# Twinklebear/tray_rust

Measured on AMD Instinct MI355X. Metric: Msamples/s (whole node) at 1920x1080; achieved HBM GB/s vs peak, higher is better.
Workload: dtype f32

## Files before the change

### tray_rust_amd/csrc/hip/dev_integrator.h

```cpp
#pragma once
#include "dev_tex.h"

#ifdef TR_LEAN_TILES
#ifndef TR_LEAN_PICK
#define TR_LEAN_MIS_PDF_FIRST
#endif
#endif

namespace tr {

template <int ANIM>
TR_DEV Ray camera_ray(const DevScene& sc, float px, float py, float time) {
    const TrayCamera& c = *sc.camera_p;
    f3 q = xf_point(c.raster_to_cam, mk(px, py, 0.0f));
    f3 px_pos = mk(c.scaling[0], c.scaling[1], c.scaling[2]) * q;
    f3 d = normalized(px_pos);
    const float frame_time = (c.shutter_close - c.shutter_open) * time + c.shutter_open;
    Ray r;
    if (ANIM && c.animated) {
        float x[TR_XF_WORDS];
        if (ANIM == 1 && sc.xf_tab) {
            const float4* __restrict__ rec = reinterpret_cast<const float4*>(sc.xf_tab + ((size_t)xf_time_index(time) * sc.xf_tab_stride + sc.n_moving) * TR_XF_REC);
#pragma unroll
            for (int q = 0; q < TR_XF_WORDS / 4; ++q) { const float4 v = rec[q]; x[4 * q] = v.x; x[4 * q + 1] = v.y; x[4 * q + 2] = v.z; x[4 * q + 3] = v.w; }
        } else
        eval_xform_stack(sc.xf_levels, sc.keyframes, sc.knots, c.xf_first, c.xf_count, frame_time, x);
        r.o = xf_point_affine_w(x, x[25], mk(0.0f, 0.0f, 0.0f));
        r.d = xf_vector(x, d);
    } else {
        r.o = xf_point(c.cam_world, mk(0.0f, 0.0f, 0.0f));
        r.d = xf_vector(c.cam_world, d);
    }
    r.min_t = 0.0f; r.max_t = TR_INF;
    r.time = frame_time; r.col = 0u;
    return r;
}

TR_DEV void pixel_sample(uint32_t kp, uint32_t s, uint32_t spp, uint32_t px, uint32_t py, float& x, float& y, float& t) {
    uint32_t idx = permute(s, spp, draw(kp, PD_PERM_XY));
    x = van_der_corput(idx, draw(kp, PD_SCR_X)) + (float)px;
    y = sobol(idx, draw(kp, PD_SCR_Y)) + (float)py;
    t = van_der_corput(permute(s, spp, draw(kp, PD_PERM_T)), draw(kp, PD_SCR_T));
}

TR_DEV float rr_draw(uint32_t ks, uint32_t bounce) { return (float)(draw(ks, SD_RR + bounce) >> 8) / 16777216.0f; }

template <int ANIM>
TR_DEV f3 inst_emission(const DevScene& sc, const TrayInstance* __restrict__ in, float time) {
    if (ANIM && in->emis_count >= 2u) return color_keys_at(sc.color_keys + in->emis_first, in->emis_count, time);
    return mk(in->emission[0], in->emission[1], in->emission[2]);
}
template <int ANIM>
TR_DEV f3 emitter_radiance(const DevScene& sc, const TrayInstance* __restrict__ in, f3 w, f3 n, float time) {
    return dot(w, n) > 0.0f ? inst_emission<ANIM>(sc, in, time) : mk(0.0f, 0.0f, 0.0f);
}

enum : uint32_t {
    LF_ALIVE = 1u,
    LF_SPECULAR = 2u,
    LF_SHADOW = 4u,
    LF_MIS = 8u,
    LF_LAST = 16u,
    LF_MIS_MISS = 1024u,
    LF_MIS_UNTESTED = 2048u
};
enum : uint32_t { WANT_NONE = 0, WANT_LIGHT = 1, WANT_MIS = 2, WANT_PATH = 3 };

struct Lane {
    uint32_t flags;
    uint32_t bounce;
    uint32_t ks;
    float time;
    uint32_t col;
    f3 d;
#define LN_O(ln) ((ln).bsdf.p)
    f3 throughput, illum;
    f3 first_ng;
    Bsdf bsdf;
    uint32_t light_inst;
    f3 li;
    union { f3 wi_l; f3 mis_f; };
    float pdf_l;
    f3 aux_d;
    f3 direct;
    f3 t_vertex;
    LdsB perm_lds = nullptr;
    uint32_t smp_kind = TRAY_SAMPLER_LOW_DISCREPANCY, smp_offset = 0u;
#ifdef TR_STAGE_CLOCKS
    unsigned long long* qclk = nullptr;
    long long qt = 0;
#endif
};
#ifdef TR_STAGE_CLOCKS
#define TR_QCLK_START(ln) do { if ((ln).qclk) (ln).qt = clock64(); } while (0)
#define TR_QCLK(ln, k) do { if ((ln).qclk) { const long long n_ = clock64(); (ln).qclk[k] += (unsigned long long)(n_ - (ln).qt); (ln).qt = n_; } } while (0)
#else
#define TR_QCLK_START(ln) ((void)0)
#define TR_QCLK(ln, k) ((void)0)
#endif

TR_DEV void lane_start_sample(Lane& ln, const Ray& cam_ray, uint32_t ks) {
    ln.flags = LF_ALIVE;
    ln.bounce = 0u;
    ln.ks = ks;
    LN_O(ln) = cam_ray.o; ln.d = cam_ray.d;
    ln.time = cam_ray.time; ln.col = 0u;
    ln.throughput = mk(1.0f, 1.0f, 1.0f);
    ln.illum = mk(0.0f, 0.0f, 0.0f);
}

TR_DEV uint32_t lane_perm_entry(const DevScene& sc, const Lane& ln, uint32_t s1, uint32_t s2) {
    const uint32_t off1 = ((s1 & (TR_PERM_POOL - 1u)) << 4) + ln.bounce;
    const uint32_t e1 = ln.perm_lds ? (uint32_t)ln.perm_lds[off1] : (uint32_t)sc.perm_pool[off1];
    const uint32_t off2 = ((s2 & (TR_PERM_POOL - 1u)) << 4) + (__brev(e1 >> 4) >> 28);
    return ln.perm_lds ? (uint32_t)ln.perm_lds[off2] : (uint32_t)sc.perm_pool[off2];
}
TR_DEV float lane_uniform(const Lane& ln, uint32_t dim, uint32_t c) {
    return (float)(draw(ln.ks, 64u + 32u * dim + 2u * ln.bounce + c) >> 8) / 16777216.0f;
}
TR_DEV void lane_2d(const DevScene& sc, const Lane& ln, uint32_t dim, float& u0, float& u1) {
    if (ln.smp_kind == TRAY_SAMPLER_UNIFORM) { u0 = lane_uniform(ln, dim, 0u); u1 = lane_uniform(ln, dim, 1u); return; }
    const uint32_t sx = draw(ln.ks, dim), sy = draw(ln.ks, dim + 1u);
    const uint32_t e = lane_perm_entry(sc, ln, sx, sy);
    if (ln.smp_kind == TRAY_SAMPLER_ADAPTIVE) {
        const uint32_t idx = (__brev(e >> 4) >> 28) + ln.smp_offset;
        u0 = van_der_corput(idx, sx); u1 = sobol(idx, sy);
        return;
    }
    u0 = u24_to_unit(((e & 0xf0u) << 24) ^ sx);
    u1 = u24_to_unit((e << 28) ^ sy);
}
TR_DEV float lane_1d(const DevScene& sc, const Lane& ln, uint32_t dim) {
    if (ln.smp_kind == TRAY_SAMPLER_UNIFORM) return lane_uniform(ln, dim, 0u);
    const uint32_t s = draw(ln.ks, dim);
    const uint32_t e = lane_perm_entry(sc, ln, s, s >> 8);
    if (ln.smp_kind == TRAY_SAMPLER_ADAPTIVE) return van_der_corput((__brev(e >> 4) >> 28) + ln.smp_offset, s);
    return u24_to_unit(((e & 0xf0u) << 24) ^ s);
}

TR_DEV Ray stage_a_ray(const Lane& ln) {
    Ray r;
    r.o = LN_O(ln); r.d = ln.d;
    r.min_t = ln.bounce == 0u ? 0.0f : 0.001f;
    r.max_t = TR_INF;
    r.time = ln.time; r.col = ln.col;
    return r;
}
TR_DEV Ray stage_b_ray(const Lane& ln) {
    Ray r;
    r.o = ln.bsdf.p; r.d = ln.aux_d; r.min_t = 0.001f; r.max_t = 0.999f;
    r.time = ln.time; r.col = ln.col;
    return r;
}
TR_DEV Ray stage_c_ray(const Lane& ln) {
    Ray r;
    r.o = ln.bsdf.p; r.d = ln.aux_d; r.min_t = 0.001f; r.max_t = TR_INF;
    r.time = ln.time; r.col = ln.col;
    return r;
}

template <int ANIM>
TR_DEV void vertex_begin(const DevScene& sc, Lane& ln, const HitRec& rec, Counters& cnt) {
    cnt.vertices++;
    const Ray ray = stage_a_ray(ln);
    Hit hit = finish_hit<ANIM>(sc, ray, rec);
    if (ln.bounce == 0u) ln.first_ng = hit.ng;
    const TrayInstance* __restrict__ inst = sc.instances + hit.inst;
    if (ln.bounce == 0u || (ln.flags & LF_SPECULAR)) {
        if (inst->kind != TRAY_INST_RECEIVER) {
            f3 w = -ln.d;
            ln.illum = ln.illum + ln.throughput * emitter_radiance<ANIM>(sc, inst, w, ln.first_ng, ln.time);
        }
    }
    ln.bsdf = make_bsdf(sc, hit);
    if (sc.integrator == TRAY_INTEGRATOR_NORMALS_DEBUG) {
        ln.illum = (ln.bsdf.n + mk(1.0f, 1.0f, 1.0f)) / 2.0f;
        ln.flags &= ~(LF_ALIVE | LF_SHADOW | LF_MIS | LF_MIS_MISS | LF_MIS_UNTESTED);
        return;
    }
    ln.direct = mk(0.0f, 0.0f, 0.0f);
    ln.t_vertex = ln.throughput;
    ln.flags &= ~(LF_SHADOW | LF_MIS | LF_LAST | LF_MIS_MISS | LF_MIS_UNTESTED);
    float l1 = lane_1d(sc, ln, SD_L1);
    float fl = l1 * (float)sc.n_lights;
    uint32_t li_idx = fl > 0.0f ? (uint32_t)fl : 0u;
    if (li_idx > sc.n_lights - 1u) li_idx = sc.n_lights - 1u;
    ln.light_inst = sc.lights[li_idx];
    const TrayInstance* __restrict__ light = sc.instances + ln.light_inst;
    f3 p_w;
    float x[TR_XF_WORDS];
    if (ANIM) instance_xf_at<ANIM>(sc, light, ln.time, ln.col, x);
    if (light->kind == TRAY_INST_POINT_EMITTER) {
        f3 pos = ANIM ? xf_point_affine_w(x, x[25], mk(0.0f, 0.0f, 0.0f)) : xf_point(light->mat, mk(0.0f, 0.0f, 0.0f));
        ln.wi_l = normalized(pos - ln.bsdf.p);
        ln.li = inst_emission<ANIM>(sc, light, ln.time) / length_sqr(pos - ln.bsdf.p);
        ln.pdf_l = 1.0f;
        p_w = pos;
    } else {
        float l2x, l2y;
        lane_2d(sc, ln, SD_L2, l2x, l2y);
        f3 p_l = ANIM ? xf_point_affine_w(x + 12, x[24], ln.bsdf.p) : xf_point(light->inv, ln.bsdf.p);
        f3 p_sampled, normal;
        geom_sample(light, p_l, l2x, l2y, p_sampled, normal);
        f3 w_il = normalized(p_sampled - p_l);
        ln.pdf_l = geom_pdf(light, p_l, w_il);
        ln.li = emitter_radiance<ANIM>(sc, light, -w_il, normal, ln.time);
        p_w = ANIM ? xf_point_affine_w(x, x[25], p_sampled) : xf_point(light->mat, p_sampled);
        ln.wi_l = ANIM ? xf_vector(x, w_il) : xf_vector(light->mat, w_il);
    }
    if (ln.pdf_l > 0.0f && !is_black(ln.li)) {
        ln.aux_d = p_w - ln.bsdf.p;
        ln.flags |= LF_SHADOW;
    }
}

// ... 192 lines not shown
```

### tray_rust_amd/csrc/hip/kernel_tiles.hip

```cpp
#ifndef TR_TILES_GROUP
#error "compile with -DTR_TILES_GROUP=<0 | 1> (csrc/Makefile)"
#endif
#define TR_DEVICE_TU
#define TR_LEAN_TILES
#include "kernels.hip"
#include "kernel_select.h"
#include "kernel_tiles.h"

namespace tr_tiles {

#if TR_TILES_GROUP == 0
void path_tiles(int feat, bool light_filter, dim3 grid, dim3 block, size_t lds, hipStream_t stream, const tr::DevScene& dev, const uint2* tiles,
                uint32_t tile_count, uint32_t chunk, uint32_t chunk_stride, uint32_t spp, uint32_t kf, uint32_t levels, float* rgbw, uint32_t* counter,
                DevStats* stats) {
    if (feat != FEAT_NONE) { path_tiles_lobes(feat, light_filter, grid, block, lds, stream, dev, tiles, tile_count, chunk, chunk_stride, spp, kf, levels, rgbw, counter, stats); return; }
    select_path_tiles_filter<0, FEAT_NONE>(light_filter, [&](auto kernel) {
        hipLaunchKernelGGL(kernel, grid, block, lds, stream, dev, tiles, tile_count, chunk, chunk_stride, spp, kf, levels, rgbw, counter, stats);
    });
}
const void* path_tiles_kernel(int feat, bool light_filter) {
    if (feat != FEAT_NONE) return path_tiles_kernel_lobes(feat, light_filter);
    const void* k = nullptr;
    select_path_tiles_filter<0, FEAT_NONE>(light_filter, [&](auto kernel) { k = reinterpret_cast<const void*>(kernel); });
    return k;
}
#else
template <class F>
static void select_lobes(int feat, bool light_filter, F&& f) {
    if (feat == FEAT_MERL) select_path_tiles_filter<0, FEAT_MERL>(light_filter, f);
    else if (feat == FEAT_SPEC) select_path_tiles_filter<0, FEAT_SPEC>(light_filter, f);
    else if (feat == (FEAT_MERL | FEAT_SPEC)) select_path_tiles_filter<0, FEAT_MERL | FEAT_SPEC>(light_filter, f);
    else if (feat == (FEAT_ALL | FEAT_TEX)) select_path_tiles_filter<0, FEAT_ALL | FEAT_TEX>(light_filter, f);
    else select_path_tiles_filter<0, FEAT_ALL>(light_filter, f);
}
void path_tiles_lobes(int feat, bool light_filter, dim3 grid, dim3 block, size_t lds, hipStream_t stream, const tr::DevScene& dev, const uint2* tiles,
                      uint32_t tile_count, uint32_t chunk, uint32_t chunk_stride, uint32_t spp, uint32_t kf, uint32_t levels, float* rgbw,
                      uint32_t* counter, DevStats* stats) {
    select_lobes(feat, light_filter, [&](auto kernel) {
        hipLaunchKernelGGL(kernel, grid, block, lds, stream, dev, tiles, tile_count, chunk, chunk_stride, spp, kf, levels, rgbw, counter, stats);
    });
}
const void* path_tiles_kernel_lobes(int feat, bool light_filter) {
    const void* k = nullptr;
    select_lobes(feat, light_filter, [&](auto kernel) { k = reinterpret_cast<const void*>(kernel); });
    return k;
}
#endif

}
```

### tray_rust_amd/csrc/hip/kernels.hip

```cpp
#ifndef TR_HOST_EMU
#include <hip/hip_runtime.h>
#endif
#include <stdint.h>

#include <cstdio>
#include <cstdlib>
#include <cstring>
#include <mutex>
#include <thread>
#include <dlfcn.h>
#include <string>
#include <type_traits>
#include <utility>
#include <algorithm>
#include <vector>

#include "../../../include/trayhip.h"
#include "../host/validate.hpp"
#include "dev_integrator.h"
#include "dev_whitted.h"

namespace trayh { void set_error(const std::string& msg); }
using trayh::set_error;
using namespace tr;
// ... 139 lines not shown
                                                       int x0, int y0, int py_l, float sx, float sy, f3 c) {
    const float img_x = sx - 0.5f, img_y = sy - 0.5f;
    const float e8 = (img_y - (float)(y0 + py_l)) * 8.0f;
    const float fl8 = floorf(e8);
    if (e8 == fl8 || fl8 < -4.0f || fl8 > 3.0f) { film_splat_global(sc, rgbw, s_table, x0, y0, sx, sy, c); return; }
    const int cy = (int)fl8 + 4;
    const int fpw = sc.fpw;
    const int xr0 = max(x0 - fpw, 0), xr1 = min(x0 + 8 + fpw, (int)sc.width - 1);
    int ix_lo, ix_hi;
    film_admit(sx, xr0, xr1, fpw, ix_lo, ix_hi);
    const int wx0 = x0 - fpw;
    float* __restrict__ row = bins + (py_l * 8 + cy) * ROW_W * 4;
    for (int ix = ix_lo; ix <= ix_hi; ++ix) {
        float fx = fabsf((float)ix - img_x) * sc.inv_w;
        if (fx > sc.filter_w) continue;
        int fx_idx = min((int)(fx * (float)TRAY_FILTER_TABLE_SIZE), TRAY_FILTER_TABLE_SIZE - 1);
        float wx = s_tx[fx_idx];
        float* __restrict__ o = row + (ix - wx0) * 4;
        if (LDS_BINS) {
            atomicAdd(o + 0, wx * c.x); atomicAdd(o + 1, wx * c.y); atomicAdd(o + 2, wx * c.z); atomicAdd(o + 3, wx);
        } else {
            wg_add(o + 0, wx * c.x); wg_add(o + 1, wx * c.y); wg_add(o + 2, wx * c.z); wg_add(o + 3, wx);
        }
    }
}

#include "wavefront.h"

TR_DEV const float* sc_filter_table(const DevScene& sc) { return sc.filter_table; }

template <int ANIM, int FEAT, int INTEG = TRAY_INTEGRATOR_PATH, bool LFILT = false>
__global__ __launch_bounds__(TR_BLOCK, (FEAT == 15 || INTEG != TRAY_INTEGRATOR_PATH) ? TR_MIN_WAVES_SIDE : ANIM ? TR_MIN_WAVES_ANIM : TR_MIN_WAVES) void k_path_tiles(const DevScene scv, const uint2* __restrict__ tiles, uint32_t tile_count,
                                                         uint32_t chunk, uint32_t chunk_stride, uint32_t spp, uint32_t kf, uint32_t levels,
                                                         float* __restrict__ rgbw, uint32_t* __restrict__ counter,
                                                         DevStats* __restrict__ stats
#ifdef TR_SAMPLE_RANGES
                                                         , uint32_t smp_begin = 0u, uint32_t smp_end = 0u
#endif
                                                         ) {
    const float* __restrict__ const s_table = sc_filter_table(scv);
    __shared__ float s_rowbin[ROWBIN_SIZE];
    __shared__ float s_tx[TRAY_FILTER_TABLE_SIZE], s_ty[TRAY_FILTER_TABLE_SIZE];
    __shared__ uint4 s_perm[TR_PERM_BYTES / 16];
    TR_DYN_LDS(uint32_t, s_stack);
    __shared__ uint32_t s_tile, s_next_sample;
    float* const s_win = reinterpret_cast<float*>(s_stack + scv.win_offset);
    const DevScene& sc = scv;
    const DevScene* const scp = &scv;
    const uint32_t tid = threadIdx.x;
    const uint32_t lane = tid & 63u;
    uint32_t* const my_stack = s_stack + tid;
    if (tid < TRAY_FILTER_TABLE_SIZE) { s_tx[tid] = sc.filter_x[tid]; s_ty[tid] = sc.filter_y[tid]; }
    s_perm[tid] = reinterpret_cast<const uint4*>(sc.perm_pool)[tid];
    static_assert(TR_PERM_BYTES / 16 == TR_BLOCK, "one uint4 of the permutation pool per thread");
    const bool film_rows = sc.film_rows != 0u;
    Counters cnt;
    cnt.rays = 0; cnt.vertices = 0;
    uint32_t w_samples = 0u, w_vertices = 0u, w_rays = 0u;
#ifdef TR_STAGE_CLOCKS
    unsigned long long clk[12] = {0, 0, 0, 0, 0, 0, 0, 0, 0, 0, 0, 0};
    long long clk_t = clock64();
#endif
    for (;;) {
        __syncthreads();
        if (tid == 0) { s_tile = atomicAdd(counter, 1u); s_next_sample = 0u; }
        if (film_rows) { for (uint32_t i = tid; i < ROWBIN_SIZE; i += TR_BLOCK) s_rowbin[i] = 0.0f; }
        else for (uint32_t i = tid; i < 4 * WIN_PLANE; i += TR_BLOCK) s_win[i] = 0.0f;
        __syncthreads();
        const uint32_t item = s_tile;
        if (item >= tile_count * levels) break;
        const uint32_t level = item / tile_count, ti = item - level * tile_count, last = levels - 1u;
#ifdef TR_SAMPLE_RANGES
        const uint32_t n_smp = smp_end ? smp_end - smp_begin : spp;
        const uint32_t s_lo = smp_begin + n_smp - (n_smp >> level), s_per_slice = (level < last ? n_smp - (n_smp >> (level + 1u)) : n_smp) - (n_smp - (n_smp >> level));
#else
        const uint32_t s_per_slice = level < last ? spp >> (level + 1u) : spp >> last, s_lo = level < last ? spp - (spp >> level) : spp - (spp >> last);
#endif
        const uint2 tile = tiles[(ti / chunk) * chunk_stride * chunk + (ti % chunk)];
        const int x0 = (int)tile.x * 8, y0 = (int)tile.y * 8;
        const uint32_t n_pairs = 64u * s_per_slice;
        bool pairs_left = true;
        uint32_t row_l = 0u;
        bool pending = false;
        float sx = 0.0f, sy = 0.0f;
#ifdef TR_SAMPLE_DUMP
        size_t dump_idx = 0; uint32_t dump_v = 0u;
#endif
        Lane ln;
        ln.flags = 0u;
        ln.illum = mk(0.0f, 0.0f, 0.0f);
        ln.perm_lds = TR_LDS_B(s_perm);
#ifdef TR_STAGE_CLOCKS
        ln.qclk = clk + 8;
#endif
        for (;;) {
            bool started = false;
            uint32_t kidx = 0u;
            const bool idle = !(ln.flags & LF_ALIVE);
            if (idle && pending) {
#ifdef TR_SAMPLE_DUMP
                if (sc.sample_dump) {
                    sc.sample_dump[2 * dump_idx] = make_float4(ln.illum.x, ln.illum.y, ln.illum.z, (float)dump_v);
                    sc.sample_dump[2 * dump_idx + 1] = make_float4(ln.throughput.x, ln.throughput.y, ln.throughput.z, (float)ln.bounce);
                }
#endif
                if (film_rows) film_splat_rows(sc, s_rowbin, s_tx, rgbw, s_table, x0, y0, (int)row_l, sx, sy, lane_result(ln));
                else film_splat(sc, s_win, s_table, x0, y0, sx, sy, lane_result(ln));
                pending = false;
            }
            const unsigned long long idle_m = __ballot(idle);
            if (pairs_left && idle_m != 0ull) {
                const uint32_t n_idle = (uint32_t)__popcll(idle_m), leader = (uint32_t)__ffsll((long long)idle_m) - 1u;
                uint32_t base = 0u;
                if (lane == leader) base = atomicAdd(&s_next_sample, n_idle);
                base = __shfl(base, (int)leader);
                pairs_left = base + n_idle < n_pairs;
                const uint32_t pair = base + (uint32_t)__popcll(idle_m & ((1ull << lane) - 1ull));
                if (idle && pair < n_pairs) {
#ifdef TR_PAIR_BY_PIXEL
                    const uint32_t pix = pair / s_per_slice, s = s_lo + (pair % s_per_slice);
#else
                    const uint32_t pix = pair & 63u, s = s_lo + (pair >> 6);
#endif
                    const uint32_t px = (uint32_t)x0 + (pix & 7u), py = (uint32_t)y0 + (pix >> 3);
                    const uint32_t kp = key_pixel(kf, py * sc.width + px);
                    float t;
                    pixel_sample(kp, s, spp, px, py, sx, sy, t);
                    lane_start_sample(ln, camera_ray<ANIM>(sc, sx, sy, t), key_sample(kp, s));
                    if (ANIM) { ln.col = xf_cache_lane(); kidx = xf_time_index(t); }
                    row_l = pix >> 3;
                    started = true;
                    pending = true;
#ifdef TR_SAMPLE_DUMP
                    dump_idx = (size_t)(py * sc.width + px) * spp + s; dump_v = 0u;
#endif
                }
            }
            if (ANIM && idle_m != 0ull) xf_cache_fill_wave(sc, started, ln.time, ln.col, kidx);
            w_samples += (uint32_t)__popcll(__ballot(started));
            if (!__any(ln.flags & LF_ALIVE)) break;
            if (INTEG == TRAY_INTEGRATOR_WHITTED) {
                Ray cam;
                cam.o = LN_O(ln); cam.d = ln.d; cam.min_t = 0.0f; cam.max_t = TR_INF; cam.time = ln.time; cam.col = ln.col;
                ln.illum = whitted_run<ANIM>(sc, scp, my_stack, cam, ln.ks, (ln.flags & LF_ALIVE) != 0u, cnt, w_vertices, w_rays);
                ln.flags &= ~LF_ALIVE;
                continue;
            }
#ifdef TR_STAGE_CLOCKS
#define TR_CLK(slot) do { const long long now_ = clock64(); clk[slot] += (unsigned long long)(now_ - clk_t); clk_t = now_; } while (0)
            TR_CLK(6);
#else
#define TR_CLK(slot) ((void)0)
#endif
#pragma nounroll
            for (int stage = 0; stage < 3; ++stage) {
                const bool alive = (ln.flags & LF_ALIVE) != 0u;
                if (LFILT && stage == 2 && alive) mis_ray_filter<ANIM>(sc, ln);
                const bool want_ray = alive && (stage == 0 || (stage == 1 && (ln.flags & LF_SHADOW)) || (stage == 2 && (ln.flags & LF_MIS)));
                TraceResult tr_;
                tr_.hit = false;
                tr_.rec.t = 0.0f; tr_.rec.inst = 0xffffffffu; tr_.rec.prim = 0u; tr_.rec.b1 = 0.0f; tr_.rec.b2 = 0.0f;
                const unsigned long long wr_ = __ballot(want_ray);
                w_rays += (uint32_t)__popcll(wr_);
                if (LFILT && stage == 2) w_rays += (uint32_t)__popcll(__ballot(alive && (ln.flags & LF_MIS_MISS) != 0u));
                if (wr_ != 0ull) {
                    const Ray r = stage == 0 ? stage_a_ray(ln) : (stage == 1 ? stage_b_ray(ln) : stage_c_ray(ln));
                    tr_ = trace<ANIM, LFILT>(scp, my_stack, r, stage == 1, want_ray);
                }
                TR_CLK(stage);
                if (stage == 0) w_vertices += (uint32_t)__popcll(__ballot(alive && tr_.hit));
#ifdef TR_SAMPLE_DUMP
                if (stage == 0 && alive && tr_.hit) ++dump_v;
#endif
                if (stage == 1) {
#ifdef TR_LEAN_MIS_PDF_FIRST
                    vertex_queries<ANIM, FEAT, KM_ALL, !LFILT>(sc, ln, tr_.hit, alive);
#else
                    vertex_queries<ANIM, FEAT>(sc, ln, tr_.hit, alive);
#endif
                } else if (alive) {
                    if (stage == 0) {
                        if (tr_.hit) vertex_begin<ANIM>(sc, ln, tr_.rec, cnt);
                        else ln.flags &= ~LF_ALIVE;
                    } else {
                        if (!vertex_end<ANIM>(sc, ln, tr_.hit, tr_.rec)) ln.flags &= ~LF_ALIVE;
                    }
                }
                TR_CLK(3 + stage);
            }
        }
        __syncthreads();
        if (film_rows) {
            for (uint32_t i = tid; i < 4 * WIN_PLANE; i += TR_BLOCK) s_win[i] = 0.0f;
            __syncthreads();
            film_resolve_rows(sc, s_rowbin, s_ty, s_win, y0, tid);
            __syncthreads();
        }
        const int wx0 = x0 - sc.fpw, wy0 = y0 - sc.fph;
        const int ww = 8 + 2 * sc.fpw + 1, wh = 8 + 2 * sc.fph + 1;
        for (int i = (int)tid; i < ww * wh; i += TR_BLOCK) {
            int wy = i / ww, wx = i - wy * ww;
            int ix = wx0 + wx, iy = wy0 + wy;
            if (ix < 0 || iy < 0 || ix >= (int)sc.width || iy >= (int)sc.height) continue;
            int o = wy * WIN_STRIDE + wx;
            float a = s_win[o + 3 * WIN_PLANE];
            if (a == 0.0f && s_win[o] == 0.0f && s_win[o + WIN_PLANE] == 0.0f && s_win[o + 2 * WIN_PLANE] == 0.0f) continue;
            float* dst = rgbw + ((size_t)iy * sc.width + ix) * 4;
            atomicAdd(dst + 0, s_win[o]);
            atomicAdd(dst + 1, s_win[o + WIN_PLANE]);
            atomicAdd(dst + 2, s_win[o + 2 * WIN_PLANE]);
            atomicAdd(dst + 3, a);
        }
    }
    if (stats) {
        if (lane == 0u) {
            atomicAdd(&stats->samples, (unsigned long long)w_samples);
            atomicAdd(&stats->vertices, (unsigned long long)w_vertices);
            atomicAdd(&stats->rays, (unsigned long long)w_rays);
        }
#ifdef TR_STAGE_CLOCKS
        if ((tid & 63u) == 0u)
            for (int k = 0; k < 11; ++k) atomicAdd(&stats->trav[k], clk[k]);
#endif
    }
}
#undef TR_CLK

#ifndef TR_DEVICE_TU
__global__ __launch_bounds__(TR_BLOCK) void k_xf_table_build(const DevScene scv, float* __restrict__ table, uint32_t stride, uint32_t index0, uint32_t n_index) {
    const DevScene& sc = scv;
    const uint32_t i = blockIdx.x * TR_BLOCK + threadIdx.x, m = blockIdx.y;
    if (i >= n_index) return;
    const uint32_t index = index0 + i;
    const TrayCamera& c = *sc.camera_p;
    const float frame_time = (c.shutter_close - c.shutter_open) * xf_index_time(index) + c.shutter_open;
    uint32_t first, count;
    if (m < sc.n_moving) { const TrayInstance* __restrict__ in = sc.instances + sc.moving_ids[m]; first = in->xf_first; count = in->xf_count; }
    else { first = c.xf_first; count = c.xf_count; }
    float x[TR_XF_WORDS];
    eval_xform_stack(sc.xf_levels, sc.keyframes, sc.knots, first, count, frame_time, x);
    float4* __restrict__ rec = reinterpret_cast<float4*>(table + ((size_t)index * stride + m) * TR_XF_REC);
#pragma unroll
    for (int q = 0; q < TR_XF_WORDS / 4; ++q) rec[q] = make_float4(x[4 * q], x[4 * q + 1], x[4 * q + 2], x[4 * q + 3]);
}
__global__ __launch_bounds__(TR_BLOCK) void k_xf_table_check(const DevScene scv, const float* __restrict__ table, uint32_t stride, uint32_t n, uint32_t* __restrict__ n_bad) {
    const DevScene& sc = scv;
    const uint32_t i = blockIdx.x * TR_BLOCK + threadIdx.x;
    if (i >= n) return;
    uint32_t h = i * 0x9E3779B1u + 0x7feb352du; h ^= h >> 16; h *= 0x846ca68bu; h ^= h >> 15;
    const uint32_t index = h & 0xffffffu, m = (h >> 24) % stride;
    const TrayCamera& c = *sc.camera_p;
    const float frame_time = (c.shutter_close - c.shutter_open) * xf_index_time(index) + c.shutter_open;
    uint32_t first, count;
    if (m < sc.n_moving) { const TrayInstance* __restrict__ in = sc.instances + sc.moving_ids[m]; first = in->xf_first; count = in->xf_count; }
    else { first = c.xf_first; count = c.xf_count; }
    float x[TR_XF_WORDS];
    eval_xform_stack(sc.xf_levels, sc.keyframes, sc.knots, first, count, frame_time, x);
    const uint32_t* __restrict__ rec = reinterpret_cast<const uint32_t*>(table + ((size_t)index * stride + m) * TR_XF_REC);
    bool bad = false;
    for (int q = 0; q < TR_XF_WORDS; ++q) bad = bad || rec[q] != __float_as_uint(x[q]);
    if (bad) atomicAdd(n_bad, 1u);
}
#endif

template <int ANIM>
__global__ __launch_bounds__(TR_BLOCK) void k_debug_intersect(const DevScene scv, uint32_t n, const TrayRay* __restrict__ rays,
                                                              TrayHit* __restrict__ hits) {
    TR_DYN_LDS(uint32_t, s_stack);
    const DevScene& sc = scv;
    const DevScene* const scp = &scv;
    const uint32_t idx = blockIdx.x * blockDim.x + threadIdx.x;
    const bool in_range = idx < n;
    const uint32_t i = in_range ? idx : 0u;
    Ray r;
    r.o = mk(rays[i].o[0], rays[i].o[1], rays[i].o[2]);
    r.d = mk(rays[i].d[0], rays[i].d[1], rays[i].d[2]);
    r.min_t = rays[i].min_t; r.max_t = rays[i].max_t; r.time = rays[i].time; r.col = 0u;
    TrayHit o;
    memset(&o, 0, sizeof o);
    TraceResult tr_ = trace<ANIM>(scp, s_stack + threadIdx.x, r, false, in_range);
    if (!in_range) return;
    const HitRec rec = tr_.rec;
    if (tr_.hit) {
        float uv[2];
        f3 dp_dv;
        Hit h = finish_hit<ANIM>(sc, r, rec, uv, &dp_dv);
        o.t = rec.t; o.inst = rec.inst; o.prim = rec.prim;
        o.p[0] = h.p.x; o.p[1] = h.p.y; o.p[2] = h.p.z;
        o.n[0] = h.n.x; o.n[1] = h.n.y; o.n[2] = h.n.z;
        o.ng[0] = h.ng.x; o.ng[1] = h.ng.y; o.ng[2] = h.ng.z;
        o.u = uv[0]; o.v = uv[1];
        o.dp_du[0] = h.dp_du.x; o.dp_du[1] = h.dp_du.y; o.dp_du[2] = h.dp_du.z;
        o.dp_dv[0] = dp_dv.x; o.dp_dv[1] = dp_dv.y; o.dp_dv[2] = dp_dv.z;
    } else {
        o.t = r.max_t; o.inst = 0xffffffffu;
    }
    hits[i] = o;
}

template <int ANIM>
__global__ __launch_bounds__(TR_BLOCK) void k_debug_sample_radiance(const DevScene scv, uint32_t n, const uint32_t* __restrict__ px,
                                                                    const uint32_t* __restrict__ py, const uint32_t* __restrict__ si,
                                                                    uint32_t spp, uint32_t kf, float* __restrict__ out) {
    TR_DYN_LDS(uint32_t, s_stack);
    const DevScene& sc = scv;
    const DevScene* const scp = &scv;
    const uint32_t idx = blockIdx.x * blockDim.x + threadIdx.x;
    const bool in_range = idx < n;
    const uint32_t i = in_range ? idx : 0u;
    Counters cnt;
    cnt.rays = 0; cnt.vertices = 0;
    const uint32_t kp = key_pixel(kf, py[i] * sc.width + px[i]);
    float sx, sy, t;
    pixel_sample(kp, si[i], spp, px[i], py[i], sx, sy, t);
    Lane ln;
    lane_start_sample(ln, camera_ray<ANIM>(sc, sx, sy, t), key_sample(kp, si[i]));
    if (!in_range) ln.flags = 0u;
    uint32_t* const my_stack = s_stack + threadIdx.x;
    if (sc.integrator == TRAY_INTEGRATOR_WHITTED) {
        Ray cam;
        cam.o = LN_O(ln); cam.d = ln.d; cam.min_t = 0.0f; cam.max_t = TR_INF; cam.time = ln.time; cam.col = ln.col;
        uint32_t wv = 0u, wr = 0u;
        ln.illum = whitted_run<ANIM>(sc, scp, my_stack, cam, ln.ks, in_range, cnt, wv, wr);
        ln.flags = 0u;
    }
    while (__any(ln.flags & LF_ALIVE)) {
#pragma nounroll
        for (int stage = 0; stage < 3; ++stage) {
            const bool alive = (ln.flags & LF_ALIVE) != 0u;
            if (stage == 2 && alive) mis_ray_filter<ANIM>(sc, ln);
            const bool want_ray = alive && (stage == 0 || (stage == 1 && (ln.flags & LF_SHADOW)) || (stage == 2 && (ln.flags & LF_MIS)));
            TraceResult tr_;
            tr_.hit = false;
            tr_.rec.t = 0.0f; tr_.rec.inst = 0xffffffffu; tr_.rec.prim = 0u; tr_.rec.b1 = 0.0f; tr_.rec.b2 = 0.0f;
            if (stage == 2 && alive && (ln.flags & LF_MIS_MISS)) cnt.rays++;
            if (__any(want_ray)) {
                if (want_ray) cnt.rays++;
                const Ray r = stage == 0 ? stage_a_ray(ln) : (stage == 1 ? stage_b_ray(ln) : stage_c_ray(ln));
                tr_ = trace<ANIM>(scp, my_stack, r, stage == 1, want_ray);
            }
// ... 263 lines not shown
```

Measured before the change: 1236.

## Fold sparse MIS rays into the next iteration's primary trace stage

After: 1273 (median of 6 runs). 3.0% higher.

```diff
diff --git a/tray_rust_amd/csrc/hip/dev_integrator.h b/tray_rust_amd/csrc/hip/dev_integrator.h
--- a/tray_rust_amd/csrc/hip/dev_integrator.h
+++ b/tray_rust_amd/csrc/hip/dev_integrator.h
@@ -4,6 +4,11 @@
 #ifdef TR_LEAN_TILES
 #ifndef TR_LEAN_PICK
 #define TR_LEAN_MIS_PDF_FIRST
+#endif
+#endif
+#ifdef TR_LEAN_FOLD_MIS_RAY
+#ifndef TR_LEAN_FOLD_MIN_LANES
+#define TR_LEAN_FOLD_MIN_LANES 8
 #endif
 #endif
 
@@ -61,6 +66,10 @@
     LF_SHADOW = 4u,
     LF_MIS = 8u,
     LF_LAST = 16u,
+#ifdef TR_LEAN_FOLD_MIS_RAY
+    LF_FOLD = 16384u,
+    LF_SIT = 32768u,
+#endif
     LF_MIS_MISS = 1024u,
     LF_MIS_UNTESTED = 2048u
 };
diff --git a/tray_rust_amd/csrc/hip/kernel_fold.h b/tray_rust_amd/csrc/hip/kernel_fold.h
--- /dev/null
+++ b/tray_rust_amd/csrc/hip/kernel_fold.h
@@ -0,0 +1,10 @@
+#pragma once
+
+namespace tr_fold {
+void path_tiles(int feat, dim3 grid, dim3 block, size_t lds, hipStream_t stream, const tr::DevScene& dev, const uint2* tiles, uint32_t tile_count,
+                uint32_t chunk, uint32_t chunk_stride, uint32_t spp, uint32_t kf, uint32_t levels, float* rgbw, uint32_t* counter, DevStats* stats);
+const void* path_tiles_kernel(int feat);
+void path_tiles_lobes(int feat, dim3 grid, dim3 block, size_t lds, hipStream_t stream, const tr::DevScene& dev, const uint2* tiles, uint32_t tile_count,
+                      uint32_t chunk, uint32_t chunk_stride, uint32_t spp, uint32_t kf, uint32_t levels, float* rgbw, uint32_t* counter, DevStats* stats);
+const void* path_tiles_kernel_lobes(int feat);
+}
diff --git a/tray_rust_amd/csrc/hip/kernel_fold.hip b/tray_rust_amd/csrc/hip/kernel_fold.hip
--- /dev/null
+++ b/tray_rust_amd/csrc/hip/kernel_fold.hip
@@ -0,0 +1,47 @@
+#ifndef TR_FOLD_GROUP
+#error "compile with -DTR_FOLD_GROUP=<0 | 1> (csrc/Makefile)"
+#endif
+#define TR_DEVICE_TU
+#define TR_LEAN_TILES
+#if !defined(TR_LEAN_PICK) && !defined(TR_LEAN_FOLD_MIS_RAY)
+#define TR_LEAN_FOLD_MIS_RAY
+#endif
+#include "kernels.hip"
+#include "kernel_fold.h"
+
+namespace tr_fold {
+
+#if TR_FOLD_GROUP == 0
+void path_tiles(int feat, dim3 grid, dim3 block, size_t lds, hipStream_t stream, const tr::DevScene& dev, const uint2* tiles, uint32_t tile_count,
+                uint32_t chunk, uint32_t chunk_stride, uint32_t spp, uint32_t kf, uint32_t levels, float* rgbw, uint32_t* counter, DevStats* stats) {
+    if (feat != FEAT_NONE) { path_tiles_lobes(feat, grid, block, lds, stream, dev, tiles, tile_count, chunk, chunk_stride, spp, kf, levels, rgbw, counter, stats); return; }
+    hipLaunchKernelGGL((k_path_tiles<0, FEAT_NONE, TRAY_INTEGRATOR_PATH, false>), grid, block, lds, stream, dev, tiles, tile_count, chunk, chunk_stride, spp, kf, levels, rgbw,
+                       counter, stats);
+}
+const void* path_tiles_kernel(int feat) {
+    if (feat != FEAT_NONE) return path_tiles_kernel_lobes(feat);
+    return reinterpret_cast<const void*>(k_path_tiles<0, FEAT_NONE, TRAY_INTEGRATOR_PATH, false>);
+}
+#else
+template <class F>
+static void select_lobes(int feat, F&& f) {
+    if (feat == FEAT_MERL) f(k_path_tiles<0, FEAT_MERL, TRAY_INTEGRATOR_PATH, false>);
+    else if (feat == FEAT_SPEC) f(k_path_tiles<0, FEAT_SPEC, TRAY_INTEGRATOR_PATH, false>);
+    else if (feat == (FEAT_MERL | FEAT_SPEC)) f(k_path_tiles<0, FEAT_MERL | FEAT_SPEC, TRAY_INTEGRATOR_PATH, false>);
+    else if (feat == (FEAT_ALL | FEAT_TEX)) f(k_path_tiles<0, FEAT_ALL | FEAT_TEX, TRAY_INTEGRATOR_PATH, false>);
+    else f(k_path_tiles<0, FEAT_ALL, TRAY_INTEGRATOR_PATH, false>);
+}
+void path_tiles_lobes(int feat, dim3 grid, dim3 block, size_t lds, hipStream_t stream, const tr::DevScene& dev, const uint2* tiles, uint32_t tile_count,
+                      uint32_t chunk, uint32_t chunk_stride, uint32_t spp, uint32_t kf, uint32_t levels, float* rgbw, uint32_t* counter, DevStats* stats) {
+    select_lobes(feat, [&](auto kernel) {
+        hipLaunchKernelGGL(kernel, grid, block, lds, stream, dev, tiles, tile_count, chunk, chunk_stride, spp, kf, levels, rgbw, counter, stats);
+    });
+}
+const void* path_tiles_kernel_lobes(int feat) {
+    const void* k = nullptr;
+    select_lobes(feat, [&](auto kernel) { k = reinterpret_cast<const void*>(kernel); });
+    return k;
+}
+#endif
+
+}
diff --git a/tray_rust_amd/csrc/hip/kernel_tiles.hip b/tray_rust_amd/csrc/hip/kernel_tiles.hip
--- a/tray_rust_amd/csrc/hip/kernel_tiles.hip
+++ b/tray_rust_amd/csrc/hip/kernel_tiles.hip
@@ -6,19 +6,27 @@
 #include "kernels.hip"
 #include "kernel_select.h"
 #include "kernel_tiles.h"
+#include "kernel_fold.h"
 
 namespace tr_tiles {
 
 #if TR_TILES_GROUP == 0
+static bool folds() { const char* e = getenv("TRAYHIP_LEAN_FOLD"); return !e || atoi(e) != 0; }
 void path_tiles(int feat, bool light_filter, dim3 grid, dim3 block, size_t lds, hipStream_t stream, const tr::DevScene& dev, const uint2* tiles,
                 uint32_t tile_count, uint32_t chunk, uint32_t chunk_stride, uint32_t spp, uint32_t kf, uint32_t levels, float* rgbw, uint32_t* counter,
                 DevStats* stats) {
+    if (!light_filter && folds()) {
+        if (getenv("TRAYHIP_STATS")) fprintf(stderr, "[trayhip] lean tile kernel: the folding instantiation (libtrayhip_foldmis.so)\n");
+        tr_fold::path_tiles(feat, grid, block, lds, stream, dev, tiles, tile_count, chunk, chunk_stride, spp, kf, levels, rgbw, counter, stats);
+        return;
+    }
     if (feat != FEAT_NONE) { path_tiles_lobes(feat, light_filter, grid, block, lds, stream, dev, tiles, tile_count, chunk, chunk_stride, spp, kf, levels, rgbw, counter, stats); return; }
     select_path_tiles_filter<0, FEAT_NONE>(light_filter, [&](auto kernel) {
         hipLaunchKernelGGL(kernel, grid, block, lds, stream, dev, tiles, tile_count, chunk, chunk_stride, spp, kf, levels, rgbw, counter, stats);
     });
 }
 const void* path_tiles_kernel(int feat, bool light_filter) {
+    if (!light_filter && folds()) return tr_fold::path_tiles_kernel(feat);
     if (feat != FEAT_NONE) return path_tiles_kernel_lobes(feat, light_filter);
     const void* k = nullptr;
     select_path_tiles_filter<0, FEAT_NONE>(light_filter, [&](auto kernel) { k = reinterpret_cast<const void*>(kernel); });
diff --git a/tray_rust_amd/csrc/hip/kernels.hip b/tray_rust_amd/csrc/hip/kernels.hip
--- a/tray_rust_amd/csrc/hip/kernels.hip
+++ b/tray_rust_amd/csrc/hip/kernels.hip
@@ -315,32 +315,76 @@
 #else
 #define TR_CLK(slot) ((void)0)
 #endif
+#ifdef TR_LEAN_FOLD_MIS_RAY
+            constexpr bool FOLD = !LFILT && !ANIM && INTEG == TRAY_INTEGRATOR_PATH;
+            if (FOLD) ln.flags &= ~LF_SIT;
+#endif
 #pragma nounroll
             for (int stage = 0; stage < 3; ++stage) {
+#ifdef TR_LEAN_FOLD_MIS_RAY
+                const bool alive = FOLD ? (ln.flags & (LF_ALIVE | LF_SIT)) == LF_ALIVE : (ln.flags & LF_ALIVE) != 0u;
+#else
                 const bool alive = (ln.flags & LF_ALIVE) != 0u;
+#endif
                 if (LFILT && stage == 2 && alive) mis_ray_filter<ANIM>(sc, ln);
                 const bool want_ray = alive && (stage == 0 || (stage == 1 && (ln.flags & LF_SHADOW)) || (stage == 2 && (ln.flags & LF_MIS)));
                 TraceResult tr_;
                 tr_.hit = false;
                 tr_.rec.t = 0.0f; tr_.rec.inst = 0xffffffffu; tr_.rec.prim = 0u; tr_.rec.b1 = 0.0f; tr_.rec.b2 = 0.0f;
+#ifdef TR_LEAN_FOLD_MIS_RAY
+                unsigned long long wr_ = __ballot(want_ray);
+                if (FOLD && stage == 2 && wr_ != 0ull && (uint32_t)__popcll(wr_) < (uint32_t)(TR_LEAN_FOLD_MIN_LANES)) {
+                    if (want_ray) {
+                        ln.flags |= LF_FOLD;
+#ifdef TR_HOST_EMU
+                        { extern unsigned long long tr_fold_rays; ++tr_fold_rays; }
+#endif
+                    }
+                    wr_ = 0ull;
+                }
+                const bool folded = FOLD && (ln.flags & LF_FOLD) != 0u;
+#else
                 const unsigned long long wr_ = __ballot(want_ray);
+#endif
                 w_rays += (uint32_t)__popcll(wr_);
                 if (LFILT && stage == 2) w_rays += (uint32_t)__popcll(__ballot(alive && (ln.flags & LF_MIS_MISS) != 0u));
                 if (wr_ != 0ull) {
+#ifdef TR_LEAN_FOLD_MIS_RAY
+                    const Ray r = stage == 0 && !folded ? stage_a_ray(ln) : (stage == 1 ? stage_b_ray(ln) : stage_c_ray(ln));
+#else
                     const Ray r = stage == 0 ? stage_a_ray(ln) : (stage == 1 ? stage_b_ray(ln) : stage_c_ray(ln));
+#endif
                     tr_ = trace<ANIM, LFILT>(scp, my_stack, r, stage == 1, want_ray);
                 }
                 TR_CLK(stage);
+#ifdef TR_LEAN_FOLD_MIS_RAY
+                if (stage == 0) w_vertices += (uint32_t)__popcll(__ballot(alive && !folded && tr_.hit));
+#ifdef TR_SAMPLE_DUMP
+                if (stage == 0 && alive && !folded && tr_.hit) ++dump_v;
+#endif
+#else
                 if (stage == 0) w_vertices += (uint32_t)__popcll(__ballot(alive && tr_.hit));
 #ifdef TR_SAMPLE_DUMP
                 if (stage == 0 && alive && tr_.hit) ++dump_v;
 #endif
+#endif
                 if (stage == 1) {
 #ifdef TR_LEAN_MIS_PDF_FIRST
                     vertex_queries<ANIM, FEAT, KM_ALL, !LFILT>(sc, ln, tr_.hit, alive);
 #else
                     vertex_queries<ANIM, FEAT>(sc, ln, tr_.hit, alive);
 #endif
+#ifdef TR_LEAN_FOLD_MIS_RAY
+                } else if (alive) {
+                    if (stage == 0 && !folded) {
+                        if (tr_.hit) vertex_begin<ANIM>(sc, ln, tr_.rec, cnt);
+                        else ln.flags &= ~LF_ALIVE;
+                    } else if (stage == 0 || !folded) {
+                        if (!vertex_end<ANIM>(sc, ln, tr_.hit, tr_.rec)) ln.flags &= ~LF_ALIVE;
+                        if (stage == 0) ln.flags = (ln.flags & ~(LF_FOLD | LF_MIS)) | LF_SIT;
+                    }
+                }
+#else
                 } else if (alive) {
                     if (stage == 0) {
                         if (tr_.hit) vertex_begin<ANIM>(sc, ln, tr_.rec, cnt);
@@ -349,6 +393,7 @@
                         if (!vertex_end<ANIM>(sc, ln, tr_.hit, tr_.rec)) ln.flags &= ~LF_ALIVE;
                     }
                 }
+#endif
                 TR_CLK(3 + stage);
             }
         }
```
